# DH-Ng/TacEx

Hardware: AMD Instinct MI355X
Metric: tactile_frames_per_sec (higher is better)
Workload: dtype f32; 1 GPU; 1024 envs x 2 GelSight Mini per GPU = 2048 frames/step/GPU, Taxim RGB 320x240 + FOTS markers (99); BASELINE configs[2] (C3); envs_per_gpu=1024, sensors_per_env=2, markers=True, sensors=group, gather=obs32 u8 (9551872 B/rank, N=1: no collective), arch=gfx950:sramecc+:xnack-

## Files before the change

tacex_amd/csrc/tacex_capi.hip:

```cpp
#include <hip/hip_runtime.h>
#include <stdarg.h>
#include <stdio.h>
#include <string.h>

#include <algorithm>
#include <string>
#include <mutex>
#include <vector>

#include "tacex_hip.h"
#include "tacex_internal.h"
#include "taxim_layout.h"

namespace tacex {

static thread_local char g_err[512] = "";

void set_error(const char* fmt, ...) {
  va_list ap;
  va_start(ap, fmt);
  vsnprintf(g_err, sizeof(g_err), fmt, ap);
  va_end(ap);
}

// ... 627 lines not shown
  if (env == 0) return B;
  if (env > 0) return env < B ? env : B;
  const bool stream = tail_route(c, true, false) == kTailStream;
  const size_t per_frame = (size_t)3 * c->H * c->W * sizeof(float);
  const size_t n = stream ? ((size_t)(per_frame <= (size_t)240 * 320 * 12 ? 2048 : 1024) * 240 * 320 * 12) / per_frame : ((size_t)240 << 20) / per_frame;
  if (n < 1 || (size_t)B < (stream ? n + n / 2 : 2 * n)) return B;
  const size_t nchunks = ((size_t)B + n - 1) / n;
  return (int)(((size_t)B + nchunks - 1) / nchunks);
}

static int level_chunk_env() { static const int env = getenv("TACEX_LEVEL_CHUNK_FRAMES") ? atoi(getenv("TACEX_LEVEL_CHUNK_FRAMES")) : -1; return env; }
static int level_chunk_frames(const tacex_taxim_ctx* c, int B) {
  const int env = level_chunk_env();
  if (env == 0) return B;
  if (env > 0) return env < B ? env : B;
  const size_t per_frame = (size_t)3 * c->H * c->W * sizeof(float);
  const size_t n = ((size_t)240 << 20) / per_frame;
  if (n < 1 || (size_t)B < n + n / 2) return B;
  const size_t nchunks = ((size_t)B + n - 1) / n;
  return (int)(((size_t)B + nchunks - 1) / nchunks);
}

int tacex_taxim_chunk_frames(const tacex_taxim_ctx* c, int B) { return (c && B > 0) ? chunk_frames(c, B) : 0; }

static int resize_obs(tacex_taxim_ctx* c, const Pass& p) {
  float* dst = p.u8 ? p.obs_scratch + obs_resize_floats(c->H, c->W, p.oh, p.ow, p.B) : static_cast<float*>(p.obs);
  HIP_TRY(run_resize_aa(p.rgb, c->H, c->W, dst, p.oh, p.ow, p.B, 3, p.obs_scratch, p.stream), "resize_aa (observation)");
  if (p.u8) HIP_TRY(run_obs_to_u8(dst, static_cast<uint8_t*>(p.obs), (size_t)p.B * p.oh * p.ow * 3, p.stream), "obs_to_u8_kernel");
  return 0;
}

struct PassState { float* z[2]; float* tmp; const float *sa, *sb, *pd; int n_fused, n_band, band_grow; bool stream_tail; };

struct LevelPlan { int frames, streams, n_chunks; bool depth_interleaved, order_early; };

static LevelPlan plan_band_levels(const tacex_taxim_ctx* c, const Pass& p, const PassState& s) {
  LevelPlan lp{};
  lp.frames = s.stream_tail ? level_chunk_frames(c, p.B) : p.B;
  static const int lvl_streams_env = getenv("TACEX_LEVEL_STREAMS") ? atoi(getenv("TACEX_LEVEL_STREAMS")) : 2;
  const int lvl_streams = lvl_streams_env > tacex_taxim_ctx::kMaxLvlStreams ? tacex_taxim_ctx::kMaxLvlStreams : lvl_streams_env;
  bool dual = s.stream_tail && lvl_streams > 1 && !c->profiling && s.n_band > 0 && lp.frames < p.B && (p.B + lp.frames - 1) / lp.frames >= 3;
  for (int l = 0; dual && l < s.n_band; ++l)
    dual = blur_level_single_kernel(c->levels[l], l == 0, c->H, c->W);
  lp.streams = dual ? lvl_streams : 1;
  if (dual && level_chunk_env() < 0) lp.frames = (lp.frames + lvl_streams - 1) / lvl_streams;
  lp.n_chunks = (p.B + lp.frames - 1) / lp.frames;
  static const int depth_min_frames = getenv("TACEX_DEPTH_INTERLEAVE_MIN_FRAMES") ? atoi(getenv("TACEX_DEPTH_INTERLEAVE_MIN_FRAMES")) : 128;
  lp.depth_interleaved = p.depth.armed && dual && lp.frames >= depth_min_frames;
  static const int order_early_env = getenv("TACEX_STREAM_ORDER_EARLY") ? atoi(getenv("TACEX_STREAM_ORDER_EARLY")) : 1;
  lp.order_early = order_early_env != 0 && s.stream_tail && dual && lvl_streams == 2 && p.rows != nullptr && lp.n_chunks >= 3;
  return lp;
}

static int run_band_levels(tacex_taxim_ctx* c, const Pass& p, const PassState& s, const LevelPlan& lp, const float** out, bool* order_done) {
  hipStream_t const st = p.stream;
  const size_t npix = (size_t)c->H * c->W;
  const bool dual = lp.streams > 1;
  if (p.depth.armed && !lp.depth_interleaved)
    if (int rc = run_depth_pass(p.depth, c->H, c->W, st)) return rc;
  if (dual) {
    if (!c->lvl_fork) HIP_TRY(hipEventCreateWithFlags(&c->lvl_fork, hipEventDisableTiming), "hipEventCreate");
    for (int q = 0; q < lp.streams - 1; ++q) {
      if (!c->lvl_stream[q] || c->lvl_caller != st)
        if (hipError_t es = level_stream(c->device, st, q, &c->lvl_stream[q]); es != hipSuccess) return fail_hip(es, "hipStreamCreate(band levels)");
      if (!c->lvl_join[q]) HIP_TRY(hipEventCreateWithFlags(&c->lvl_join[q], hipEventDisableTiming), "hipEventCreate");
    }
    c->lvl_caller = st;
    HIP_TRY(hipEventRecord(c->lvl_fork, st), "hipEventRecord");
    for (int q = 0; q < lp.streams - 1; ++q) HIP_TRY(hipStreamWaitEvent(c->lvl_stream[q], c->lvl_fork, 0), "hipStreamWaitEvent");
  }
  const StreamPlan* tail_plan = nullptr;
  bool order_early = lp.order_early;
  if (order_early) {
    const bool want_obs = p.obs_scratch && p.obs;
    if (int rc = stream_plan(c, s.n_fused, p.B, want_obs ? p.oh : 0, want_obs ? p.ow : 0, &tail_plan)) return rc;
    if (p.B * tail_plan->nstrips * tail_plan->nseg > c->stream_order_cap) order_early = false;
  }
  if (order_early && !lp.depth_interleaved)
    HIP_TRY(run_stream_order(c->levels, c->n_levels, s.n_fused, *tail_plan, p.B, c->H, p.rows, s.band_grow, c->stream_order, c->lvl_stream[0], order_done),
            "stream_order_kernel");
  const float* src = nullptr;
  for (int b0 = 0, chunk_no = 0; b0 < p.B; b0 += lp.frames, ++chunk_no) {
    const Pass q = p.slice(b0, p.B - b0 < lp.frames ? p.B - b0 : lp.frames);
    const int lane = dual ? chunk_no % lp.streams : 0;
    hipStream_t const cst = lane > 0 ? c->lvl_stream[lane - 1] : st;
    if (lp.depth_interleaved) {
      if (int rc = run_depth_pass(q.depth, c->H, c->W, cst)) return rc;
      if (order_early && chunk_no == lp.n_chunks - 2) {
        if (!c->order_evt) HIP_TRY(hipEventCreateWithFlags(&c->order_evt, hipEventDisableTiming), "hipEventCreate");
        HIP_TRY(hipEventRecord(c->order_evt, cst), "hipEventRecord");
      } else if (order_early && chunk_no == lp.n_chunks - 1) {
        HIP_TRY(hipStreamWaitEvent(cst, c->order_evt, 0), "hipStreamWaitEvent");
        HIP_TRY(run_stream_order(c->levels, c->n_levels, s.n_fused, *tail_plan, p.B, c->H, p.rows, s.band_grow, c->stream_order, cst, order_done),
                "stream_order_kernel");
      }
    }
    src = nullptr;
    int grow = 0, grow_x = 0;
    for (int l = 0; l < s.n_band; ++l) {
      const bool last = l == c->n_levels - 1;
      float* dst = (last && p.z_out) ? p.z_out : s.z[l & 1];
      StageTimer t(c, cst, 1 + l);
      HIP_TRY(run_blur_level(c->levels[l], src ? src + b0 * npix : nullptr, q.hm, c->gel_dev, s.sa + b0, s.sb + b0, s.pd + b0, dst + b0 * npix,
                             s.tmp, last ? q.mask_out : nullptr, q.B, c->H, c->W, c->contact_scale, last ? 0 : 1, l == 0, cst, q.rows, grow, grow_x),
              "blur level");
      grow += (c->levels[l].kh - 1) / 2;
      grow_x += (c->levels[l].kw - 1) / 2;
      src = dst;
    }
  }
  if (dual) {
    for (int q = 0; q < lp.streams - 1; ++q) {
      HIP_TRY(hipEventRecord(c->lvl_join[q], c->lvl_stream[q]), "hipEventRecord");
      HIP_TRY(hipStreamWaitEvent(st, c->lvl_join[q], 0), "hipStreamWaitEvent");
    }
  }
  *out = src;
  return 0;
}

static int end_stream_tail(tacex_taxim_ctx* c, const Pass& p, const PassState& s, const float* src, bool order_done) {
  StageTimer t(c, p.stream, c->n_levels + 2);
  const bool want_obs = p.obs_scratch && p.obs;
  const StreamPlan* plan = nullptr;
  if (int rc = stream_plan(c, s.n_fused, p.B, want_obs ? p.oh : 0, want_obs ? p.ow : 0, &plan)) return rc;
  const bool fuse_obs = want_obs && plan->obs_ready &&
                        (size_t)p.B * plan->nstrips * plan->nseg * plan->obs_nrows * plan->obs_ncols * 3 <= obs_resize_floats(c->H, c->W, p.oh, p.ow, p.B);
  const bool pix = p.frame0 >= 0 && c->fots_pix_z && c->mk_x;
  float* z_last = src == s.z[0] ? s.z[1] : s.z[0];
  const int n_items = p.B * plan->nstrips * plan->nseg;
  HIP_TRY(run_stream_tail(c->levels, c->n_levels, s.n_fused, src, p.hm, c->gel_dev, s.sa, s.sb, s.pd, &c->shade, p.rgb, z_last, p.B, c->H, c->W,
                          c->contact_scale, *plan, fuse_obs ? p.obs_scratch : nullptr, p.fots_part,
                          (int)(tail_tiles_per_frame(c->H, c->W) * kTailWavesPerTile),
                          pix ? c->fots_pix_z + (size_t)p.frame0 * c->fots_taps.n_markers : nullptr,
                          pix ? c->fots_pix_m + (size_t)p.frame0 * c->fots_taps.n_markers : nullptr, p.stream, p.rows, s.band_grow,
                          n_items <= c->stream_order_cap ? c->stream_order : nullptr, order_done),
          "taxim_stream_kernel");
  if (fuse_obs) HIP_TRY(run_obs_finish_stream(p.obs_scratch, p.obs, p.u8, *plan, p.B, p.stream), "obs_finish_stream_kernel");
  else if (want_obs) return resize_obs(c, p);
  return 0;
}

static int end_tiled_tail(tacex_taxim_ctx* c, const Pass& p, const PassState& s, const float* src) {
  StageTimer t(c, p.stream, c->n_levels + 2);
  bool fuse_obs = false;
  int onry = 0, oncx = 0, oky = 0, okx = 0;
  if (p.obs_scratch && p.obs && p.rgb) {
    if (int rc = ensure_obs_tables(c, p.oh, p.ow)) return rc;
    const int k0 = c->levels[c->n_levels - s.n_fused].kw;
    fuse_obs = obs_fusable(c->obs_tab, c->H, c->W, s.n_fused, k0) && tail_obs_geom(s.n_fused, k0, &onry, &oncx, &oky, &okx) &&
               obs_part_floats(c->H, c->W, p.B, onry, oncx) <= obs_resize_floats(c->H, c->W, p.oh, p.ow, p.B);
  }
  const bool pix = p.frame0 >= 0 && c->fots_pix_z;
  HIP_TRY(run_tail(c->levels, c->n_levels, s.n_fused, src, p.hm, c->gel_dev, s.sa, s.sb, s.pd, p.z_out, p.mask_out, &c->shade, p.rgb,
                   fuse_obs ? p.obs_scratch : nullptr, fuse_obs ? &c->obs_tab : nullptr, p.fots_part, pix ? &c->fots_taps : nullptr,
                   pix ? c->fots_pix_z + (size_t)p.frame0 * c->fots_taps.n_markers : nullptr,
                   (p.frame0 >= 0 && c->fots_pix_m) ? c->fots_pix_m + (size_t)p.frame0 * c->fots_taps.n_markers : nullptr, p.B, c->H, c->W,
// ... 225 lines not shown
```

tacex_amd/csrc/tacex_internal.h:

```cpp
#pragma once
#include <hip/hip_runtime.h>
#include <stdint.h>

namespace tacex {

struct LevelDesc {
  int kw = 1, kh = 1;
  bool gel_zero = false;
  bool same_taps = false;
  float* taps_w_dev = nullptr;
  float* taps_h_dev = nullptr;
  float* taps_mfma_dev = nullptr;
  float* taps_pad_dev = nullptr;
};

struct FotsReduce {
  float zmax;
  int count;
  int sum_row;
  int sum_col;
};
constexpr int kTailWavesPerTile = 8;
constexpr int kTailMaxMarkersPerTile = 16;
struct FotsTaps {
  const int* mk_tile = nullptr;
  const int* mk_cnt = nullptr;
  int n_markers = 0;
};

struct ShadeParams {
  int H = 0, W = 0, nb = 0, calib_h = 0, calib_w = 0;
  float pixmm = 0.f, x_binr = 0.f, y_binr = 0.f;
  float* poly_dev = nullptr;
  float* bg_nhwc_dev = nullptr;
  float* fx_dev = nullptr;
  float* fy_dev = nullptr;
  float* flat_rgb_dev = nullptr;
};

hipError_t run_frame_min(const float* in, bool from_depth, float* hm_out, float* fmin, float* indent,
                         uint8_t* cam_u8, int B, int npix, float near_mm, float far_m, float far_mm, float gelpad_h,
                         float gelpad_dmin, hipStream_t st);
hipError_t run_indenter_height_map(const float* desc, float* hm, float* fmin, float* indent, int B, int H, int W, float pixmm,
                                   float gel_top_mm, float far_clip_mm, float gelpad_h, float gelpad_dmin, hipStream_t st);
hipError_t run_press_depth(const float* fmin, const float* press, float* sa, float* sb, float* pd, int B,
                           int no_shift, hipStream_t st);
enum BlurRoute { kRouteGeneric = 0, kRouteBand = 1, kRouteBandLoop384 = 2, kRouteBandLoop640 = 3, kRouteMfma = 4 };
BlurRoute blur_level_route(const LevelDesc& lv, bool first, int H, int W);
bool blur_level_single_kernel(const LevelDesc& lv, bool first, int H, int W);
hipError_t run_blur_level(const LevelDesc& lv, const float* src, const float* hm, const float* gel,
                          const float* sa, const float* sb, const float* pd, float* dst, float* tmp,
                          uint8_t* mask_out, int B, int H, int W, float contact_scale, int restore,
                          bool first, hipStream_t st, const int* rows_ext = nullptr, int ext_grow = 0, int ext_grow_x = 0);
bool frame_rows_supported(int H, int W);
hipError_t run_fill_rows(int* rows, int B, int H, int W, hipStream_t st);
hipError_t run_frame_rows(const float* in, bool from_depth, float* hm_out, float* fmin, float* indent, uint8_t* cam_u8,
                          const float* press_in, int* rows_out, int B, int H, int W, float near_mm, float far_m, float far_mm,
                          float gelpad_h, float gelpad_dmin, hipStream_t st);
hipError_t run_shade(const ShadeParams& sp, const float* z, float* rgb, uint8_t* idx_out, int B,
                     hipStream_t st);
hipError_t run_resize_aa(const float* src, int sh, int sw, float* dst, int dh, int dw, int B, int C, float* tmp,
                         hipStream_t st);

struct ShadowParams {
  bool ready = false;
  int ndir = 0, nfan = 0, nheight = 0, nstep = 0;
  int wl = 0, wr = 0, wt = 0, wb = 0;
  float depth0 = 0.4f, height_prec = 0.1f, disc_prec = 0.1f, step_x = 0.f, step_y = 0.f;
  float* fan_dev = nullptr;
  float* fan_cos_dev = nullptr;
  float* fan_sin_dev = nullptr;
  float* table_dev = nullptr;
  int sblur_kw = 1, sblur_kh = 1, final_kw = 1, final_kh = 1;
  float* sblur_taps_w_dev = nullptr; float* sblur_taps_h_dev = nullptr;
  float* final_taps_w_dev = nullptr; float* final_taps_h_dev = nullptr;
};
hipError_t run_shadow_rays(const ShadowParams& sw, const ShadeParams& sp, const float* z, const uint8_t* mask, const float* gel,
                           const float* gdir, float* shadow_min, int B, hipStream_t st);
hipError_t run_shadow(const ShadowParams& sw, const ShadeParams& sp, const float* z, const uint8_t* mask, const float* gel,
                      float* rgb, float* ws_raw, float* ws_shadow, float* ws_gdir, float* ws_tmp, int B, hipStream_t st);

__host__ __device__ inline int mfma_h_window_col(int KS, int g, int ks) {
  const int p = (ks >> 2) + (g >> 1) * (KS >> 2);
  return 4 * (4 * (p >> 1) + (p & 1) + 2 * (g & 1)) + (ks & 3);
}
__host__ __device__ inline int mfma_h_row(int i) { return (i >= 4 && i < 12) ? 2 * (i - 4) + 1 : 2 * (i < 4 ? i : i - 8); }

int tail_levels(const LevelDesc* lv, int n_levels, int H, int W);
struct ObsTables {
  const int* ylo; const int* ycnt; const float* ysum; const float* wy; int ky;
  const int* xlo; const int* xcnt; const float* xsum; const float* wx; int kx;
  int oh, ow;
  int ymax, xmax;
};
hipError_t run_tail(const LevelDesc* lv, int n_levels, int n_fused, const float* zin, const float* hm, const float* gel,
                    const float* sa, const float* sb, const float* pd, float* z_out, uint8_t* mask_out,
                    const ShadeParams* sp, float* rgb, float* obs_part, const ObsTables* obs_tab, FotsReduce* fots_part,
                    const FotsTaps* taps, float* pix_z, uint8_t* pix_m, int B, int H, int W, float contact_scale, hipStream_t st);
size_t tail_tiles_per_frame(int H, int W);
hipError_t run_obs_finish(const float* part, void* obs, bool u8, const ObsTables& t, int H, int W, int B, int nry, int ncx,
                          hipStream_t st);
bool tail_obs_geom(int n_fused, int k0, int* nry, int* ncx, int* ky, int* kx);
hipError_t run_obs_to_u8(const float* src, uint8_t* dst, size_t n, hipStream_t st);
size_t obs_part_floats(int H, int W, int B, int nry, int ncx);
bool obs_fusable(const ObsTables& t, int H, int W, int n_fused, int k0);

constexpr int kStreamMaxLevels = 5;
constexpr int kStreamMaxSeg = 8;
struct StreamRowInfo {
  float fy;
  int o0;
  float w0, w1, w2;
  int mk0, mk1;
  int pad;
};
constexpr int kStreamRowInts = 32;
constexpr int kStreamMkSlots = 20;
struct StreamPlan {
  int nstrips = 0, strip_w = 0, nseg = 0, seg_rows = 0;
  int lv_nstrips = 0, lv_strip_w = 0, lv_nseg = 0, lv_seg_rows = 0;
  bool obs_ready = false;
  ObsTables obs{};
  const void* rows = nullptr;
  int obs_kxp = 0;
  const int* obs_strip_q0 = nullptr; const int* obs_strip_nq = nullptr;
  const int* obs_seg_oa = nullptr; const int* obs_seg_ob = nullptr;
  int obs_nrows = 0, obs_ncols = 0;
  const int* mk_x = nullptr; const int* mk_id = nullptr; int n_markers = 0;
  bool mk_vec = false;
};
int stream_obs_lds_floats();
int stream_obs_max_cols();
bool stream_supported(int n_fused, int k0, int H, int W);
bool stream_geometry(int n_fused, int k0, int W, int* nstrips, int* strip_w, int* lv_nstrips, int* lv_strip_w);
int stream_segments(int B, int nstrips, int H, int warm_rows, int waves_per_simd);
int stream_warm_rows(int n_fused, int k0, bool levels_kernel);
int stream_waves_per_simd(int n_fused, int k0);
hipError_t run_stream_flat_image(const ShadeParams* sp, int H, int W, hipStream_t st);
hipError_t run_stream_tail(const LevelDesc* lv, int n_levels, int n_fused, const float* zin, const float* hm, const float* gel,
                           const float* sa, const float* sb, const float* pd, const ShadeParams* sp, float* rgb, float* z_last,
                           int B, int H, int W, float contact_scale, const StreamPlan& plan, float* obs_part,
                           FotsReduce* fots_part, int fots_stride, float* pix_z, uint8_t* pix_m, hipStream_t st, const int* rows_ext = nullptr, int ext_grow = 0,
                           int* order_buf = nullptr,
                           bool order_done = false);
hipError_t run_stream_order(const LevelDesc* lv, int n_levels, int n_fused, const StreamPlan& plan, int B, int H, const int* rows_ext, int ext_grow,
                            int* order_buf, hipStream_t st, bool* launched);
hipError_t run_obs_finish_stream(const float* part, void* obs, bool u8, const StreamPlan& plan, int B, hipStream_t st);

inline hipError_t ensure_dynamic_lds(const void* kern, size_t lds, size_t (&granted)[64]) {
  if (lds <= 48 * 1024) return hipSuccess;
  int dev = 0;
  if (hipGetDevice(&dev) != hipSuccess || dev < 0 || dev >= 64) dev = 0;
  if (lds <= granted[dev]) return hipSuccess;
  hipError_t e = hipFuncSetAttribute(kern, hipFuncAttributeMaxDynamicSharedMemorySize, (int)lds);
  if (e == hipSuccess) granted[dev] = lds;
  return e;
}

inline hipError_t dynamic_lds_limit(const void* kern, size_t (&avail)[64], size_t* limit) {
  int dev = 0;
  if (hipGetDevice(&dev) != hipSuccess || dev < 0 || dev >= 64) dev = 0;
  if (!avail[dev]) {
    hipFuncAttributes a{};
    const hipError_t e = hipFuncGetAttributes(&a, kern);
    if (e != hipSuccess) return e;
    avail[dev] = a.sharedSizeBytes < 160 * 1024 ? 160 * 1024 - a.sharedSizeBytes : 1;
  }
  *limit = avail[dev];
  return hipSuccess;
}

void set_error(const char* fmt, ...);
int fail_hip(hipError_t e, const char* what);

}
```

tacex_amd/csrc/taxim_blur.h:

```cpp
#pragma once
#include <hip/hip_runtime.h>
#include <stdint.h>

namespace tacex {

struct BlurArgs {
  const float* src;
  const float* hm;
  const float* gel;
  const float* shift_a;
  const float* shift_b;
  const float* pdepth;
  float* dst;
  uint8_t* mask_out;
  const float* taps;
  int H, W, B;
  int pitch;
  int padx;
  float contact_scale;
  int restore;
  int row0, nbands;
  const int* rows_ext;
  int ext_grow;
  int ext_grow_x;
};

bool mfma_supported(int k, bool first, int H, int W);
hipError_t dispatch_mfma(int k, bool first, const BlurArgs& a, hipStream_t st);

}
```

tacex_amd/csrc/taxim_kernels.hip:

```cpp
#include <hip/hip_runtime.h>
#include <stdint.h>
#include <stdlib.h>

#include <type_traits>

#include "tacex_internal.h"
#include "taxim_device.h"
#include "taxim_blur.h"

namespace tacex {

template <bool FROM_DEPTH>
__global__ __launch_bounds__(1024) void frame_min_kernel(
    const float* __restrict__ in, float* __restrict__ hm_out, float* __restrict__ fmin_out,
    float* __restrict__ indent_out, uint8_t* __restrict__ cam_u8, int npix, float nmm, float far_m, float fmm,
    float gelpad_h, float gelpad_dmin) {
  const int b = blockIdx.x;
  const float* src = in + (size_t)b * npix;
  float m = INFINITY;
  const int n4 = npix >> 2;
  for (int i = threadIdx.x; i < n4; i += blockDim.x) {
    v4f v = reinterpret_cast<const v4f*>(src)[i];
    if (FROM_DEPTH) {
#pragma unroll
// ... 841 lines not shown
hipError_t run_fill_rows(int* rows, int B, int H, int W, hipStream_t st) {
  hipLaunchKernelGGL(fill_rows_kernel, dim3((B + 255) / 256), dim3(256), 0, st, rows, B, H, W);
  return hipGetLastError();
}
hipError_t run_frame_rows(const float* in, bool from_depth, float* hm_out, float* fmin, float* indent, uint8_t* cam_u8,
                          const float* press_in, int* rows_out, int B, int H, int W, float near_mm, float far_m, float far_mm,
                          float gelpad_h, float gelpad_dmin, hipStream_t st) {
  const int w4 = W >> 2;
  int nt = w4 <= 1024 ? (1024 / w4) * w4 : 1024;
  if (nt < 512 || (nt & 63)) nt = 1024;
  if (from_depth)
    hipLaunchKernelGGL(frame_rows_kernel<true>, dim3(B), dim3(nt), 0, st, in, hm_out, fmin, indent, cam_u8, press_in, rows_out,
                       H, W, near_mm, far_m, far_mm, gelpad_h, gelpad_dmin);
  else
    hipLaunchKernelGGL(frame_rows_kernel<false>, dim3(B), dim3(nt), 0, st, in, hm_out, fmin, indent, cam_u8, press_in, rows_out,
                       H, W, near_mm, far_m, far_mm, gelpad_h, gelpad_dmin);
  return hipGetLastError();
}

hipError_t run_frame_min(const float* in, bool from_depth, float* hm_out, float* fmin, float* indent,
                         uint8_t* cam_u8, int B, int npix, float near_mm, float far_m, float far_mm, float gelpad_h,
                         float gelpad_dmin, hipStream_t st) {
  if (from_depth)
    hipLaunchKernelGGL(frame_min_kernel<true>, dim3(B), dim3(1024), 0, st, in, hm_out, fmin, indent, cam_u8,
                       npix, near_mm, far_m, far_mm, gelpad_h, gelpad_dmin);
  else
    hipLaunchKernelGGL(frame_min_kernel<false>, dim3(B), dim3(1024), 0, st, in, hm_out, fmin, indent, cam_u8,
                       npix, near_mm, far_m, far_mm, gelpad_h, gelpad_dmin);
  return hipGetLastError();
}

hipError_t run_press_depth(const float* fmin, const float* press, float* sa, float* sb, float* pd, int B,
                           int no_shift, hipStream_t st) {
  hipLaunchKernelGGL(press_depth_kernel, dim3((B + 255) / 256), dim3(256), 0, st, fmin, press, sa, sb, pd, B,
                     no_shift);
  return hipGetLastError();
}

BlurRoute blur_level_route(const LevelDesc& lv, bool first, int H, int W) {
  if (lv.same_taps && lv.taps_mfma_dev && mfma_supported(lv.kw, first, H, W)) return kRouteMfma;
  const bool unrolled_ok = band_supported(lv.kw, H, W) && (!first || band_first_supported(lv.kw));
  if (lv.same_taps && lv.taps_pad_dev && band_loop_supported(lv.kw, H, W) && (!unrolled_ok || lv.kw >= band_loop_min_k()) &&
      (band_loop_min_k() != 35 || !unrolled_ok))
    return W <= 384 ? kRouteBandLoop384 : kRouteBandLoop640;
  if (lv.same_taps && unrolled_ok) return kRouteBand;
  return kRouteGeneric;
}

bool blur_level_single_kernel(const LevelDesc& lv, bool first, int H, int W) { return blur_level_route(lv, first, H, W) == kRouteMfma; }

hipError_t run_blur_level(const LevelDesc& lv, const float* src, const float* hm, const float* gel,
                          const float* sa, const float* sb, const float* pd, float* dst, float* tmp,
                          uint8_t* mask_out, int B, int H, int W, float contact_scale, int restore,
                          bool first, hipStream_t st, const int* rows_ext, int ext_grow, int ext_grow_x) {
  const BlurRoute route = blur_level_route(lv, first, H, W);
  if (route == kRouteMfma) {
    BlurArgs a{};
    a.src = src; a.hm = hm; a.shift_a = sa; a.shift_b = sb; a.pdepth = pd;
    a.rows_ext = lv.gel_zero ? rows_ext : nullptr; a.ext_grow = ext_grow; a.ext_grow_x = ext_grow_x;
    a.gel = lv.gel_zero ? nullptr : gel;
    a.dst = dst; a.mask_out = mask_out; a.taps = lv.taps_mfma_dev; a.H = H; a.W = W; a.B = B;
    a.contact_scale = contact_scale; a.restore = restore;
    return dispatch_mfma(lv.kw, first, a, st);
  }
  if (route == kRouteBandLoop384 || route == kRouteBandLoop640) {
    BlurArgs a{};
    a.src = src; a.hm = hm; a.gel = gel; a.shift_a = sa; a.shift_b = sb; a.pdepth = pd;
    a.dst = dst; a.mask_out = mask_out; a.taps = lv.taps_pad_dev; a.H = H; a.W = W; a.B = B;
    a.contact_scale = contact_scale; a.restore = restore;
    if (route == kRouteBandLoop384) return first ? launch_band_loop<true, 384>(a, lv.kw, st) : launch_band_loop<false, 384>(a, lv.kw, st);
    return first ? launch_band_loop<true, 640>(a, lv.kw, st) : launch_band_loop<false, 640>(a, lv.kw, st);
  }
  if (route == kRouteBand) {
    BlurArgs a{};
    a.src = src; a.hm = hm; a.gel = gel; a.shift_a = sa; a.shift_b = sb; a.pdepth = pd;
    a.dst = dst; a.mask_out = mask_out; a.taps = lv.taps_w_dev; a.H = H; a.W = W; a.B = B;
    a.contact_scale = contact_scale; a.restore = restore;
    return dispatch_band(lv.kw, first, a, st);
  }
  GenericArgs g{};
  g.hm = hm; g.gel = gel; g.shift_a = sa; g.shift_b = sb; g.pdepth = pd; g.H = H; g.W = W; g.B = B;
  g.contact_scale = contact_scale;
  const size_t n = (size_t)B * H * W;
  const int grid = (int)((n + 255) / 256 < 65536 ? (n + 255) / 256 : 65536);
  g.src = src; g.dst = tmp; g.taps = lv.taps_h_dev; g.k = lv.kh; g.first = first ? 1 : 0; g.restore = 0;
  g.mask_out = nullptr;
  hipLaunchKernelGGL(blur_generic_v_kernel, dim3(grid), dim3(256), 0, st, g);
  g.src = tmp; g.dst = dst; g.taps = lv.taps_w_dev; g.k = lv.kw; g.first = 0; g.restore = restore;
  g.mask_out = mask_out;
  hipLaunchKernelGGL(blur_generic_h_kernel, dim3(grid), dim3(256), 0, st, g);
  return hipGetLastError();
}

hipError_t run_shade(const ShadeParams& sp, const float* z, float* rgb, uint8_t* idx_out, int B,
                     hipStream_t st) {
  ShadeArgs a{};
  a.z = z; a.poly = sp.poly_dev; a.bg = sp.bg_nhwc_dev; a.fx = sp.fx_dev; a.fy = sp.fy_dev; a.rgb = rgb;
  a.idx_out = idx_out; a.H = sp.H; a.W = sp.W; a.B = B; a.nb = sp.nb; a.pixmm = sp.pixmm;
  a.calib_h = (float)sp.calib_h; a.calib_w = (float)sp.calib_w;
  a.x_binr = sp.x_binr; a.y_binr = sp.y_binr;
  a.gsy = (float)(0.5 * sp.H / sp.calib_h / (double)sp.pixmm); a.gsx = (float)(0.5 * sp.W / sp.calib_w / (double)sp.pixmm);
  a.inv_x_binr = (float)(1.0 / (double)sp.x_binr); a.inv_y_binr = (float)(1.0 / (double)sp.y_binr);
  const int npix = sp.H * sp.W;
  hipLaunchKernelGGL(shade_kernel, dim3((npix + 255) / 256, B), dim3(256), 0, st, a);
  return hipGetLastError();
}

hipError_t run_resize_aa(const float* src, int sh, int sw, float* dst, int dh, int dw, int B, int C, float* tmp,
                         hipStream_t st) {
  if (tmp) {
    const size_t n1 = (size_t)B * dh * sw * C, n2 = (size_t)B * dh * dw * C;
    const int g1 = (int)((n1 + 255) / 256 < 65536 ? (n1 + 255) / 256 : 65536);
// ... 19 lines not shown
```

tacex_amd/csrc/taxim_mfma.hip:

```cpp
#include <hip/hip_runtime.h>
#include <stdint.h>
#include <stdlib.h>

#include "tacex_internal.h"
#include "taxim_blur.h"
#include "taxim_device.h"

namespace tacex {

typedef float f32x4 __attribute__((ext_vector_type(4)));
#ifndef TACEX_MFMA_CH
#define TACEX_MFMA_CH 4
#endif
#ifndef TACEX_MFMA_FENCE
#define TACEX_MFMA_FENCE 0
#endif
#ifndef TACEX_MFMA_H_CONSEC
#define TACEX_MFMA_H_CONSEC 0
#endif

template <int K, bool FIRST, int NTILE, bool GZ>
__global__ __launch_bounds__(640) void blur_mfma_kernel(BlurArgs a) {
  constexpr int TH = 16 * NTILE;
  constexpr int R = (K - 1) / 2, RA = (R + 7) & ~7, WIN = 16 + 2 * RA, KS = WIN / 4;
  constexpr int KU = KS + 4 * (NTILE - 1);
#ifndef TACEX_MFMA_CH61
#define TACEX_MFMA_CH61 TACEX_MFMA_CH
#endif
#ifndef TACEX_MFMA_CH117
#define TACEX_MFMA_CH117 TACEX_MFMA_CH
#endif
  constexpr int CH = K == 61 ? TACEX_MFMA_CH61 : (K == 117 ? TACEX_MFMA_CH117 : TACEX_MFMA_CH), NCH = KU / CH;
  static_assert(KU % CH == 0 && KS % 4 == 0, "window");
  extern __shared__ __attribute__((aligned(16))) char smem_raw[];
  float* mid = reinterpret_cast<float*>(smem_raw);
  const int H = a.H, W = a.W, pitch = a.pitch;
  const int lid = xcd_remap(blockIdx.x, gridDim.x);
  const int frame = lid / a.nbands;
  const int band = lid - frame * a.nbands;
  const int by0 = min(a.row0 + band * TH, H - TH);
  const size_t fo = (size_t)frame * H * W;
  const float* __restrict__ src = FIRST ? a.hm + fo : a.src + fo;
  const float* __restrict__ hm = a.hm + fo;
  const float* __restrict__ gel = a.gel;
  if constexpr (GZ) {
    if (a.rows_ext != nullptr) {
      const int lo = a.rows_ext[4 * frame] - a.ext_grow, hi = a.rows_ext[4 * frame + 1] + a.ext_grow;
      if (by0 - R > hi || by0 + TH - 1 + R < lo) {
        const int w4 = W >> 2;
        for (int i = threadIdx.x; i < TH * w4; i += blockDim.x) {
          const int r = i / w4, c = i - r * w4;
          reinterpret_cast<v4f*>(a.dst + fo + (size_t)(by0 + r) * W)[c] = (v4f)(0.0f);
          if (a.mask_out) reinterpret_cast<uchar4*>(a.mask_out + fo + (size_t)(by0 + r) * W)[c] = (uchar4){0, 0, 0, 0};
        }
        return;
      }
    }
  }
  const float sa = a.shift_a[frame], sb = a.shift_b[frame];
  const int lane = threadIdx.x & 63;
  const int wid = __builtin_amdgcn_readfirstlane((int)(threadIdx.x >> 6));
  const int li = lane & 15, g = lane >> 4;
  const int c0 = wid << 6;
#ifndef TACEX_MFMA_BLOCK_SKIP_MIN_K
#define TACEX_MFMA_BLOCK_SKIP_MIN_K 0
#endif
  bool v_need = true, h_need = true;
  if constexpr (GZ && K >= TACEX_MFMA_BLOCK_SKIP_MIN_K) {
    if (a.rows_ext != nullptr) {
      const int in_lo = a.rows_ext[4 * frame + 2] - a.ext_grow_x, in_hi = a.rows_ext[4 * frame + 3] + a.ext_grow_x;
      v_need = !(c0 + 63 < in_lo || c0 > in_hi);
      h_need = !(c0 + 63 < in_lo - R || c0 > in_hi + R);
#ifdef TACEX_MFMA_NO_BLOCK_SKIP
      v_need = h_need = true;
#endif
    }
  }

  {
    float wl[KS];
    static_for<0, KS>([&](auto kc) {
      constexpr int ks = decltype(kc)::value;
      wl[ks] = a.taps[ks * 64 + lane];
    });
    f32x4 acc[NTILE][4];
#pragma unroll
    for (int t = 0; t < NTILE; ++t)
#pragma unroll
      for (int v = 0; v < 4; ++v) acc[t][v] = (f32x4)(0.0f);
    const int rb = by0 - RA + g;
    const unsigned coff = (unsigned)(c0 + 4 * li);
    v4f xb[2][CH], gb[FIRST ? 2 : 1][FIRST ? CH : 1];
    auto issue = [&](auto chunk_c) {
      constexpr int chunk = decltype(chunk_c)::value;
      static_for<0, CH>([&](auto cc) {
        constexpr int c = decltype(cc)::value;
        int yy = reflect_idx(rb + 4 * (chunk * CH + c), H);
        yy = yy < 0 ? 0 : (yy >= H ? H - 1 : yy);
        const unsigned off = (unsigned)yy * (unsigned)W + coff;
        xb[chunk & 1][c] = *reinterpret_cast<const v4f*>(src + off);
        if constexpr (FIRST) gb[chunk & 1][c] = GZ ? (v4f)(0.0f) : *reinterpret_cast<const v4f*>(gel + off);
      });
    };
    if (v_need) {
    issue(std::integral_constant<int, 0>{});
    static_for<0, NCH>([&](auto chunk_c) {
      constexpr int chunk = decltype(chunk_c)::value;
      if constexpr (TACEX_MFMA_FENCE) __builtin_amdgcn_sched_barrier(0);
      if constexpr (chunk + 1 < NCH) issue(std::integral_constant<int, chunk + 1>{});
      if constexpr (TACEX_MFMA_FENCE) __builtin_amdgcn_sched_barrier(0);
      static_for<0, CH>([&](auto cc) {
        constexpr int c = decltype(cc)::value;
        constexpr int ku = chunk * CH + c;
        v4f x = xb[chunk & 1][c];
        if constexpr (FIRST) {
          const v4f gq = gb[chunk & 1][c];
          x.x = fminf((x.x - sa) - sb, gq.x); x.y = fminf((x.y - sa) - sb, gq.y);
          x.z = fminf((x.z - sa) - sb, gq.z); x.w = fminf((x.w - sa) - sb, gq.w);
        }
        static_for<0, NTILE>([&](auto tc) {
          constexpr int t = decltype(tc)::value;
          constexpr int ks = ku - 4 * t;
          if constexpr (ks >= 0 && ks < KS) {
            const float w = wl[ks];
            acc[t][0] = __builtin_amdgcn_mfma_f32_16x16x4f32(w, x.x, acc[t][0], 0, 0, 0);
            acc[t][1] = __builtin_amdgcn_mfma_f32_16x16x4f32(w, x.y, acc[t][1], 0, 0, 0);
            acc[t][2] = __builtin_amdgcn_mfma_f32_16x16x4f32(w, x.z, acc[t][2], 0, 0, 0);
            acc[t][3] = __builtin_amdgcn_mfma_f32_16x16x4f32(w, x.w, acc[t][3], 0, 0, 0);
          }
        });
      });
    });
    }
    const int cx = c0 + 4 * li;
#pragma unroll
    for (int t = 0; t < NTILE; ++t)
#pragma unroll
      for (int r = 0; r < 4; ++r) {
        float* rowp = mid + (16 * t + 4 * g + r) * pitch + RA;
        const float e[4] = {acc[t][0][r], acc[t][1][r], acc[t][2][r], acc[t][3][r]};
        *reinterpret_cast<v4f*>(rowp + cx) = (v4f){e[0], e[1], e[2], e[3]};
        if (cx <= RA) {
#pragma unroll
          for (int v = 0; v < 4; ++v)
            if (cx + v >= 1 && cx + v <= RA) rowp[-(cx + v)] = e[v];
        }
        if (cx + 3 >= W - 1 - RA) {
#pragma unroll
          for (int v = 0; v < 4; ++v)
            if (cx + v >= W - 1 - RA && cx + v <= W - 2) rowp[2 * (W - 1) - (cx + v)] = e[v];
        }
      }
  }
  __syncthreads();
  {
    float wl[KS];
    static_for<0, KS>([&](auto kc) {
      constexpr int ks = decltype(kc)::value;
      wl[ks] = a.taps[((TACEX_MFMA_H_CONSEC ? 0 : KS) + ks) * 64 + lane];
    });
    const float thr = -a.pdepth[frame] * a.contact_scale;
    if (!h_need) {
#pragma unroll
      for (int t = 0; t < NTILE; ++t) {
        const int hrow = TACEX_MFMA_H_CONSEC ? li : mfma_h_row(li);
        const size_t p0 = (size_t)(by0 + 16 * t + hrow) * W + c0 + 4 * g;
#pragma unroll
        for (int n = 0; n < 4; ++n) {
          *reinterpret_cast<v4f*>(a.dst + fo + p0 + 16 * n) = (v4f)(0.0f);
          if (a.mask_out) *reinterpret_cast<uchar4*>(a.mask_out + fo + p0 + 16 * n) = (uchar4){0, 0, 0, 0};
        }
      }
      return;
    }
#pragma unroll
    for (int t = 0; t < NTILE; ++t) {
      f32x4 acc[4];
#pragma unroll
      for (int n = 0; n < 4; ++n) acc[n] = (f32x4)(0.0f);
      const int hrow = TACEX_MFMA_H_CONSEC ? li : mfma_h_row(li);
      const size_t p0 = (size_t)(by0 + 16 * t + hrow) * W + c0 + 4 * g;
      v4f hv[4], gv[4];
#pragma unroll
      for (int n = 0; n < 4; ++n) {
        hv[n] = *reinterpret_cast<const v4f*>(hm + p0 + 16 * n);
        gv[n] = GZ ? (v4f)(0.0f) : *reinterpret_cast<const v4f*>(gel + p0 + 16 * n);
      }
      if constexpr (TACEX_MFMA_H_CONSEC) {
        const float* arow = mid + (16 * t + li) * pitch + g + c0;
        static_for<0, KS>([&](auto kc) {
          constexpr int ks = decltype(kc)::value;
          float q[4];
#pragma unroll
          for (int n = 0; n < 4; ++n) q[n] = arow[16 * n + 4 * ks];
#pragma unroll
          for (int n = 0; n < 4; ++n) acc[n] = __builtin_amdgcn_mfma_f32_16x16x4f32(wl[ks], q[n], acc[n], 0, 0, 0);
        });
      } else {
        const float* arow = mid + (16 * t + hrow) * pitch + c0;
        static_for<0, KS / 4>([&](auto mc) {
          constexpr int m = decltype(mc)::value;
          const int hcol = mfma_h_window_col(KS, g, 4 * m);
          v4f q[4];
#pragma unroll
          for (int n = 0; n < 4; ++n) q[n] = *reinterpret_cast<const v4f*>(arow + 16 * n + hcol);
#pragma unroll
          for (int n = 0; n < 4; ++n) acc[n] = __builtin_amdgcn_mfma_f32_16x16x4f32(wl[4 * m], q[n].x, acc[n], 0, 0, 0);
#pragma unroll
          for (int n = 0; n < 4; ++n) acc[n] = __builtin_amdgcn_mfma_f32_16x16x4f32(wl[4 * m + 1], q[n].y, acc[n], 0, 0, 0);
#pragma unroll
          for (int n = 0; n < 4; ++n) acc[n] = __builtin_amdgcn_mfma_f32_16x16x4f32(wl[4 * m + 2], q[n].z, acc[n], 0, 0, 0);
#pragma unroll
          for (int n = 0; n < 4; ++n) acc[n] = __builtin_amdgcn_mfma_f32_16x16x4f32(wl[4 * m + 3], q[n].w, acc[n], 0, 0, 0);
        });
      }
#pragma unroll
      for (int n = 0; n < 4; ++n) {
        v4f o;
        uint8_t mk[4];
#pragma unroll
        for (int k = 0; k < 4; ++k) {
          const float S = (hv[n][k] - sa) - sb;
          const float J = fminf(S, gv[n][k]);
          const bool M = ((J - gv[n][k]) < thr) && (S < 0.0f);
          o[k] = (a.restore && M) ? J : acc[n][k];
          mk[k] = M ? 1 : 0;
        }
        *reinterpret_cast<v4f*>(a.dst + fo + p0 + 16 * n) = o;
        if (a.mask_out) *reinterpret_cast<uchar4*>(a.mask_out + fo + p0 + 16 * n) = (uchar4){mk[0], mk[1], mk[2], mk[3]};
      }
    }
  }
}

template <int K, bool FIRST, int NTILE, bool GZ>
static hipError_t launch_mfma_tiles(BlurArgs a, int row0, int nbands, hipStream_t st) {
  constexpr int TH = 16 * NTILE, R = (K - 1) / 2, RA = (R + 7) & ~7;
  a.row0 = row0;
  a.nbands = nbands;
  a.padx = RA;
  a.pitch = a.W + 2 * RA + 4;
  if (((a.pitch >> 2) & 1) == 0) a.pitch += 4;
  static const size_t lds_pad = getenv("TACEX_MFMA_LDS_PAD") ? (size_t)atoi(getenv("TACEX_MFMA_LDS_PAD")) * 1024 : 0;
  const size_t lds = (size_t)TH * a.pitch * sizeof(float) + lds_pad;
  auto kern = blur_mfma_kernel<K, FIRST, NTILE, GZ>;
  static size_t granted[64] = {};
  if (hipError_t e = ensure_dynamic_lds(reinterpret_cast<const void*>(kern), lds, granted); e != hipSuccess) return e;
  hipLaunchKernelGGL(kern, dim3(nbands * a.B), dim3(a.W), lds, st, a);
  return hipGetLastError();
}

#ifndef TACEX_MFMA_NT117
#define TACEX_MFMA_NT117 1
#endif
#ifndef TACEX_MFMA_NT61
#define TACEX_MFMA_NT61 1
#endif
template <int K, bool FIRST>
static hipError_t launch_mfma(const BlurArgs& a, hipStream_t st) {
  constexpr int NT = K == 117 ? TACEX_MFMA_NT117 : (K == 61 ? TACEX_MFMA_NT61 : 1);
  if (NT > 1 && a.H % (16 * NT) == 0 && a.W > 320) {
    if (a.gel == nullptr) return launch_mfma_tiles<K, FIRST, NT, true>(a, 0, a.H / (16 * NT), st);
    return launch_mfma_tiles<K, FIRST, NT, false>(a, 0, a.H / (16 * NT), st);
  }
  if (a.gel == nullptr) return launch_mfma_tiles<K, FIRST, 1, true>(a, 0, a.H / 16, st);
  return launch_mfma_tiles<K, FIRST, 1, false>(a, 0, a.H / 16, st);
}

static int mfma_enabled() {
  static int v = -1;
  if (v < 0) { const char* e = getenv("TACEX_BLUR_MFMA"); v = e ? atoi(e) : 1; }
  return v;
}

bool mfma_supported(int k, bool first, int H, int W) {
  if (!mfma_enabled() || W % 64 != 0 || W < 64 || W > 640 || H % 16 != 0) return false;
  const int R = (k - 1) / 2;
  if (R >= H || R > W - 1 || ((R + 7) & ~7) >= W) return false;
  if (first) return k == 61 || k == 117;
  return k == 117 || k == 61 || k == 33 || k == 17 || k == 15 || k == 9;
}

hipError_t dispatch_mfma(int k, bool first, const BlurArgs& a, hipStream_t st) {
  if (first) return k == 117 ? launch_mfma<117, true>(a, st) : launch_mfma<61, true>(a, st);
  switch (k) {
    case 117: return launch_mfma<117, false>(a, st);
    case 61: return launch_mfma<61, false>(a, st);
    case 33: return launch_mfma<33, false>(a, st);
    case 17: return launch_mfma<17, false>(a, st);
    case 15: return launch_mfma<15, false>(a, st);
    case 9: return launch_mfma<9, false>(a, st);
    default: return hipErrorInvalidValue;
  }
}

}
```

tacex_amd/csrc/taxim_stream.hip:

```cpp
#include <hip/hip_runtime.h>
#include <stdint.h>
#include <stdlib.h>

#include <type_traits>
#include <vector>

#include "tacex_internal.h"
#include "taxim_device.h"

namespace tacex {

constexpr int kStreamPx = 3;
constexpr int kStreamWaves = 4;
constexpr int kStreamObsActive = 3;

struct StreamArgs {
  const float* zin;
  const float* hm;
  const float* gel;
  const float* shift_a;
  const float* shift_b;
  const float* pdepth;
  const float* taps[kStreamMaxLevels];
  ShadeArgs sh;
// ... 1064 lines not shown
  const dim3 grid(nwg);
  static const size_t lds_pad = getenv("TACEX_STREAM_LDS_PAD") ? (size_t)atoi(getenv("TACEX_STREAM_LDS_PAD")) : 0;
  const size_t lds = C::lds_bytes() + lds_pad;
  auto kern = taxim_stream_kernel<GZ, ROLE, C::min_waves(), KS...>;
  static size_t granted[64] = {};
  if (hipError_t e = ensure_dynamic_lds(reinterpret_cast<const void*>(kern), lds, granted); e != hipSuccess) return e;
  hipLaunchKernelGGL(kern, grid, dim3(64 * kStreamWaves), lds, st, a);
  return hipGetLastError();
}

template <int ROLE, int... KS>
static hipError_t launch_stream(const StreamArgs& a, bool gel_zero, hipStream_t st) {
  return gel_zero ? launch_stream_k<true, ROLE, KS...>(a, st) : launch_stream_k<false, ROLE, KS...>(a, st);
}

static void fill_shade_args(ShadeArgs& sh, const ShadeParams* sp, float* rgb, int B, int H, int W) {
  sh.poly = sp->poly_dev; sh.bg = sp->bg_nhwc_dev; sh.fx = sp->fx_dev; sh.fy = sp->fy_dev; sh.rgb = rgb;
  sh.idx_out = nullptr; sh.H = H; sh.W = W; sh.B = B; sh.nb = sp->nb; sh.pixmm = sp->pixmm;
  sh.calib_h = (float)sp->calib_h; sh.calib_w = (float)sp->calib_w; sh.x_binr = sp->x_binr; sh.y_binr = sp->y_binr;
  sh.gsy = (float)(0.5 * H / sp->calib_h / (double)sp->pixmm); sh.gsx = (float)(0.5 * W / sp->calib_w / (double)sp->pixmm);
  sh.inv_x_binr = (float)(1.0 / (double)sp->x_binr); sh.inv_y_binr = (float)(1.0 / (double)sp->y_binr);
}

hipError_t run_stream_flat_image(const ShadeParams* sp, int H, int W, hipStream_t st) {
  if (!sp->flat_rgb_dev) return hipErrorInvalidValue;
  ShadeArgs sh{};
  fill_shade_args(sh, sp, nullptr, 1, H, W);
  hipLaunchKernelGGL(stream_flat_image_kernel, dim3((W + 255) / 256, H), dim3(256), 0, st, sh, sp->flat_rgb_dev);
  return hipGetLastError();
}

static bool stream_sorted() {
  static const int sorted = getenv("TACEX_STREAM_ORDER") ? atoi(getenv("TACEX_STREAM_ORDER")) : 1;
  return sorted != 0;
}

static hipError_t launch_stream_order(int v, const int* rows_ext, int ext_grow, int B, int nstrips, int nseg, int seg_rows, int H, int* order_buf,
                                      hipStream_t st) {
  hipLaunchKernelGGL(stream_order_kernel, dim3(1), dim3(1024), 0, st, rows_ext, B * nstrips * nseg, nstrips * nseg, nseg, seg_rows, H,
                     ext_grow + variant_sum_r(v) + 1, order_buf);
  return hipGetLastError();
}

hipError_t run_stream_order(const LevelDesc* lv, int n_levels, int n_fused, const StreamPlan& plan, int B, int H, const int* rows_ext, int ext_grow,
                            int* order_buf, hipStream_t st, bool* launched) {
  *launched = false;
  if (stream_split() || !stream_sorted() || !order_buf || !lv[0].gel_zero || !rows_ext) return hipSuccess;
  const hipError_t e = launch_stream_order(stream_variant(n_fused, lv[n_levels - n_fused].kw), rows_ext, ext_grow, B, plan.nstrips, plan.nseg,
                                           plan.seg_rows, H, order_buf, st);
  *launched = e == hipSuccess;
  return e;
}

hipError_t run_stream_tail(const LevelDesc* lv, int n_levels, int n_fused, const float* zin, const float* hm, const float* gel,
                           const float* sa, const float* sb, const float* pd, const ShadeParams* sp, float* rgb, float* z_last,
                           int B, int H, int W, float contact_scale, const StreamPlan& plan, float* obs_part,
                           FotsReduce* fots_part, int fots_stride, float* pix_z, uint8_t* pix_m, hipStream_t st,
                           const int* rows_ext, int ext_grow, int* order_buf, bool order_done) {
  const bool sorted = stream_sorted();
  StreamArgs a{};
  a.rows_ext = lv[0].gel_zero ? rows_ext : nullptr; a.ext_grow = ext_grow;
  a.zin = zin; a.hm = hm; a.gel = lv[0].gel_zero ? nullptr : gel; a.shift_a = sa; a.shift_b = sb; a.pdepth = pd;
  a.H = H; a.W = W; a.B = B; a.contact_scale = contact_scale;
  for (int i = 0; i < n_fused; ++i) a.taps[i] = lv[n_levels - n_fused + i].taps_w_dev;
  fill_shade_args(a.sh, sp, rgb, B, H, W);
#ifndef TACEX_STREAM_NO_TRIM
  a.flat_rgb = sp->flat_rgb_dev;
#endif
  {
    const double t1 = tan((double)sp->x_binr) * (1.0 - 2e-5);
    a.mag0_t2 = (float)(t1 * t1);
  }
  a.rows = static_cast<const int*>(plan.rows); a.mk_vec = plan.mk_vec ? 1 : 0;
  StreamArgs sh = a;
  sh.nstrips = plan.nstrips; sh.strip_w = plan.strip_w; sh.nseg = plan.nseg; sh.seg_rows = plan.seg_rows;
  if (obs_part && plan.obs_ready) {
    sh.obs_part = obs_part;
    sh.obs_kxp = plan.obs_kxp;
    sh.obs_xlo = plan.obs.xlo; sh.obs_xcnt = plan.obs.xcnt; sh.obs_wx = plan.obs.wx; sh.obs_kx = plan.obs.kx;
    sh.obs_strip_q0 = plan.obs_strip_q0; sh.obs_strip_nq = plan.obs_strip_nq;
    sh.obs_seg_oa = plan.obs_seg_oa; sh.obs_seg_ob = plan.obs_seg_ob;
    sh.obs_nrows = plan.obs_nrows; sh.obs_ncols = plan.obs_ncols;
  }
  StreamArgs lvl = a;
  lvl.nstrips = plan.lv_nstrips; lvl.strip_w = plan.lv_strip_w; lvl.nseg = plan.lv_nseg; lvl.seg_rows = plan.lv_seg_rows;
  StreamArgs& f = stream_split() ? lvl : sh;
  f.fots_part = fots_part; f.fots_stride = fots_stride;
  if (pix_z && pix_m && plan.mk_x) {
    f.pix_z = pix_z; f.pix_m = pix_m; f.n_markers = plan.n_markers;
    f.mk_x = plan.mk_x; f.mk_id = plan.mk_id;
  }
  const int v = stream_variant(n_fused, lv[n_levels - n_fused].kw);
  const bool gz = lv[0].gel_zero;
  if (!stream_split()) {
    if (order_done) {
      sh.order = order_buf;
    } else if (sorted && order_buf && gz && rows_ext) {
      if (hipError_t e = launch_stream_order(v, rows_ext, ext_grow, B, sh.nstrips, sh.nseg, sh.seg_rows, H, order_buf, st); e != hipSuccess) return e;
      sh.order = order_buf;
    }
    if (v == 0) return launch_stream<kStreamFused, 9, 5, 3, 5>(sh, gz, st);
    if (v == 1) return launch_stream<kStreamFused, 9, 5, 9>(sh, gz, st);
    if (v == 2) return launch_stream<kStreamFused, 5, 3, 5>(sh, gz, st);
    return hipErrorInvalidValue;
  }
  if (!z_last) return hipErrorInvalidValue;
// ... 30 lines not shown
```

Measured before the change: 703,700 frames/s.

## Skip out-of-contact loads and zero-band writes in MFMA band blur levels

Adds a default-on lean variant of the MFMA blur kernel that uses buffer loads with an out-of-range offset, so source and height-map reads outside each frame's contact row/column range return zero without touching memory. When the next consumer is known to respect the contact range, blocks lying wholly outside it return early instead of writing zero bands. The aim is to cut memory traffic on mostly empty frames. The cost is an extra template instantiation, more per-lane predicate logic, and a correctness dependence on downstream kernels never reading the unwritten bands.

```diff
diff --git a/tacex_amd/csrc/tacex_capi.hip b/tacex_amd/csrc/tacex_capi.hip
--- a/tacex_amd/csrc/tacex_capi.hip
+++ b/tacex_amd/csrc/tacex_capi.hip
@@ -703,6 +703,11 @@
   return lp;
 }
 
+static bool band_lean() {
+  static const bool v = !(getenv("TACEX_BAND_LEAN") && atoi(getenv("TACEX_BAND_LEAN")) == 0);
+  return v;
+}
+
 static int run_band_levels(tacex_taxim_ctx* c, const Pass& p, const PassState& s, const LevelPlan& lp, const float** out, bool* order_done) {
   hipStream_t const st = p.stream;
   const size_t npix = (size_t)c->H * c->W;
@@ -751,9 +756,15 @@
     for (int l = 0; l < s.n_band; ++l) {
       const bool last = l == c->n_levels - 1;
       float* dst = (last && p.z_out) ? p.z_out : s.z[l & 1];
+      const bool lean = band_lean() && q.rows && c->levels[l].gel_zero;
+      bool unread = lean && dst != p.z_out && !last;
+      if (unread && l + 1 < s.n_band)
+        unread = c->levels[l + 1].gel_zero && blur_level_single_kernel(c->levels[l + 1], false, c->H, c->W);
+      else if (unread)
+        unread = s.stream_tail && stream_tail_range_aware(c->levels);
       StageTimer t(c, cst, 1 + l);
       HIP_TRY(run_blur_level(c->levels[l], src ? src + b0 * npix : nullptr, q.hm, c->gel_dev, s.sa + b0, s.sb + b0, s.pd + b0, dst + b0 * npix,
-                             s.tmp, last ? q.mask_out : nullptr, q.B, c->H, c->W, c->contact_scale, last ? 0 : 1, l == 0, cst, q.rows, grow, grow_x),
+                             s.tmp, last ? q.mask_out : nullptr, q.B, c->H, c->W, c->contact_scale, last ? 0 : 1, l == 0, cst, q.rows, grow, grow_x, lean, unread),
               "blur level");
       grow += (c->levels[l].kh - 1) / 2;
       grow_x += (c->levels[l].kw - 1) / 2;
diff --git a/tacex_amd/csrc/tacex_internal.h b/tacex_amd/csrc/tacex_internal.h
--- a/tacex_amd/csrc/tacex_internal.h
+++ b/tacex_amd/csrc/tacex_internal.h
@@ -51,7 +51,8 @@
 hipError_t run_blur_level(const LevelDesc& lv, const float* src, const float* hm, const float* gel,
                           const float* sa, const float* sb, const float* pd, float* dst, float* tmp,
                           uint8_t* mask_out, int B, int H, int W, float contact_scale, int restore,
-                          bool first, hipStream_t st, const int* rows_ext = nullptr, int ext_grow = 0, int ext_grow_x = 0);
+                          bool first, hipStream_t st, const int* rows_ext = nullptr, int ext_grow = 0, int ext_grow_x = 0, bool lean = false,
+                          bool zero_bands_unread = false);
 bool frame_rows_supported(int H, int W);
 hipError_t run_fill_rows(int* rows, int B, int H, int W, hipStream_t st);
 hipError_t run_frame_rows(const float* in, bool from_depth, float* hm_out, float* fmin, float* indent, uint8_t* cam_u8,
@@ -132,6 +133,7 @@
 int stream_obs_lds_floats();
 int stream_obs_max_cols();
 bool stream_supported(int n_fused, int k0, int H, int W);
+bool stream_tail_range_aware(const LevelDesc* lv);
 bool stream_geometry(int n_fused, int k0, int W, int* nstrips, int* strip_w, int* lv_nstrips, int* lv_strip_w);
 int stream_segments(int B, int nstrips, int H, int warm_rows, int waves_per_simd);
 int stream_warm_rows(int n_fused, int k0, bool levels_kernel);
diff --git a/tacex_amd/csrc/taxim_blur.h b/tacex_amd/csrc/taxim_blur.h
--- a/tacex_amd/csrc/taxim_blur.h
+++ b/tacex_amd/csrc/taxim_blur.h
@@ -23,6 +23,8 @@
   const int* rows_ext;
   int ext_grow;
   int ext_grow_x;
+  int lean;
+  int zero_bands_unread;
 };
 
 bool mfma_supported(int k, bool first, int H, int W);
diff --git a/tacex_amd/csrc/taxim_kernels.hip b/tacex_amd/csrc/taxim_kernels.hip
--- a/tacex_amd/csrc/taxim_kernels.hip
+++ b/tacex_amd/csrc/taxim_kernels.hip
@@ -917,12 +917,13 @@
 hipError_t run_blur_level(const LevelDesc& lv, const float* src, const float* hm, const float* gel,
                           const float* sa, const float* sb, const float* pd, float* dst, float* tmp,
                           uint8_t* mask_out, int B, int H, int W, float contact_scale, int restore,
-                          bool first, hipStream_t st, const int* rows_ext, int ext_grow, int ext_grow_x) {
+                          bool first, hipStream_t st, const int* rows_ext, int ext_grow, int ext_grow_x, bool lean, bool zero_bands_unread) {
   const BlurRoute route = blur_level_route(lv, first, H, W);
   if (route == kRouteMfma) {
     BlurArgs a{};
     a.src = src; a.hm = hm; a.shift_a = sa; a.shift_b = sb; a.pdepth = pd;
     a.rows_ext = lv.gel_zero ? rows_ext : nullptr; a.ext_grow = ext_grow; a.ext_grow_x = ext_grow_x;
+    a.lean = (lean && a.rows_ext) ? 1 : 0; a.zero_bands_unread = (a.lean && zero_bands_unread) ? 1 : 0;
     a.gel = lv.gel_zero ? nullptr : gel;
     a.dst = dst; a.mask_out = mask_out; a.taps = lv.taps_mfma_dev; a.H = H; a.W = W; a.B = B;
     a.contact_scale = contact_scale; a.restore = restore;
diff --git a/tacex_amd/csrc/taxim_mfma.hip b/tacex_amd/csrc/taxim_mfma.hip
--- a/tacex_amd/csrc/taxim_mfma.hip
+++ b/tacex_amd/csrc/taxim_mfma.hip
@@ -19,8 +19,10 @@
 #define TACEX_MFMA_H_CONSEC 0
 #endif
 
-template <int K, bool FIRST, int NTILE, bool GZ>
+template <int K, bool FIRST, int NTILE, bool GZ, bool LEAN>
 __global__ __launch_bounds__(640) void blur_mfma_kernel(BlurArgs a) {
+  static_assert(GZ || !LEAN, "the lean loads need J = min(S, 0)");
+  constexpr unsigned kNoLoad = 0x80000000u;
   constexpr int TH = 16 * NTILE;
   constexpr int R = (K - 1) / 2, RA = (R + 7) & ~7, WIN = 16 + 2 * RA, KS = WIN / 4;
   constexpr int KU = KS + 4 * (NTILE - 1);
@@ -44,9 +46,11 @@
   const float* __restrict__ hm = a.hm + fo;
   const float* __restrict__ gel = a.gel;
   if constexpr (GZ) {
-    if (a.rows_ext != nullptr) {
+    if (LEAN || a.rows_ext != nullptr) {
       const int lo = a.rows_ext[4 * frame] - a.ext_grow, hi = a.rows_ext[4 * frame + 1] + a.ext_grow;
       if (by0 - R > hi || by0 + TH - 1 + R < lo) {
+        if constexpr (LEAN)
+          if (a.zero_bands_unread) return;
         const int w4 = W >> 2;
         for (int i = threadIdx.x; i < TH * w4; i += blockDim.x) {
           const int r = i / w4, c = i - r * w4;
@@ -65,9 +69,17 @@
 #ifndef TACEX_MFMA_BLOCK_SKIP_MIN_K
 #define TACEX_MFMA_BLOCK_SKIP_MIN_K 0
 #endif
+  int ct_lo = 0, ct_hi = 0, ct_clo = 0, ct_chi = 0;
+  __amdgpu_buffer_rsrc_t src_rs, hm_rs;
+  if constexpr (LEAN) {
+    ct_lo = a.rows_ext[4 * frame]; ct_hi = a.rows_ext[4 * frame + 1];
+    ct_clo = a.rows_ext[4 * frame + 2]; ct_chi = a.rows_ext[4 * frame + 3];
+    src_rs = __builtin_amdgcn_make_buffer_rsrc(const_cast<float*>(src), 0, H * W * (int)sizeof(float), 0x00020000);
+    hm_rs = __builtin_amdgcn_make_buffer_rsrc(const_cast<float*>(hm), 0, H * W * (int)sizeof(float), 0x00020000);
+  }
   bool v_need = true, h_need = true;
   if constexpr (GZ && K >= TACEX_MFMA_BLOCK_SKIP_MIN_K) {
-    if (a.rows_ext != nullptr) {
+    if (LEAN || a.rows_ext != nullptr) {
       const int in_lo = a.rows_ext[4 * frame + 2] - a.ext_grow_x, in_hi = a.rows_ext[4 * frame + 3] + a.ext_grow_x;
       v_need = !(c0 + 63 < in_lo || c0 > in_hi);
       h_need = !(c0 + 63 < in_lo - R || c0 > in_hi + R);
@@ -91,6 +103,9 @@
     const int rb = by0 - RA + g;
     const unsigned coff = (unsigned)(c0 + 4 * li);
     v4f xb[2][CH], gb[FIRST ? 2 : 1][FIRST ? CH : 1];
+    const int vr_lo = ct_lo - a.ext_grow, vr_hi = ct_hi + a.ext_grow;
+    const bool vcol = LEAN & ((int)coff + 3 >= ct_clo - a.ext_grow_x) & ((int)coff <= ct_chi + a.ext_grow_x);
+    bool vin[2][(LEAN && FIRST) ? CH : 1];
     auto issue = [&](auto chunk_c) {
       constexpr int chunk = decltype(chunk_c)::value;
       static_for<0, CH>([&](auto cc) {
@@ -98,7 +113,13 @@
         int yy = reflect_idx(rb + 4 * (chunk * CH + c), H);
         yy = yy < 0 ? 0 : (yy >= H ? H - 1 : yy);
         const unsigned off = (unsigned)yy * (unsigned)W + coff;
-        xb[chunk & 1][c] = *reinterpret_cast<const v4f*>(src + off);
+        if constexpr (LEAN) {
+          const bool in = vcol & (yy >= vr_lo) & (yy <= vr_hi);
+          xb[chunk & 1][c] = __builtin_bit_cast(v4f, __builtin_amdgcn_raw_buffer_load_b128(src_rs, in ? off * 4u : kNoLoad, 0, 0));
+          if constexpr (FIRST) vin[chunk & 1][c] = in;
+        } else {
+          xb[chunk & 1][c] = *reinterpret_cast<const v4f*>(src + off);
+        }
         if constexpr (FIRST) gb[chunk & 1][c] = GZ ? (v4f)(0.0f) : *reinterpret_cast<const v4f*>(gel + off);
       });
     };
@@ -117,6 +138,10 @@
           const v4f gq = gb[chunk & 1][c];
           x.x = fminf((x.x - sa) - sb, gq.x); x.y = fminf((x.y - sa) - sb, gq.y);
           x.z = fminf((x.z - sa) - sb, gq.z); x.w = fminf((x.w - sa) - sb, gq.w);
+          if constexpr (LEAN) {
+            const bool in = vin[chunk & 1][c];
+            x.x = in ? x.x : 0.0f; x.y = in ? x.y : 0.0f; x.z = in ? x.z : 0.0f; x.w = in ? x.w : 0.0f;
+          }
         }
         static_for<0, NTILE>([&](auto tc) {
           constexpr int t = decltype(tc)::value;
@@ -181,9 +206,19 @@
       const int hrow = TACEX_MFMA_H_CONSEC ? li : mfma_h_row(li);
       const size_t p0 = (size_t)(by0 + 16 * t + hrow) * W + c0 + 4 * g;
       v4f hv[4], gv[4];
+      const int orow = by0 + 16 * t + hrow;
+      const bool hrow_in = LEAN & (orow >= ct_lo) & (orow <= ct_hi);
+      bool hin[4];
 #pragma unroll
       for (int n = 0; n < 4; ++n) {
-        hv[n] = *reinterpret_cast<const v4f*>(hm + p0 + 16 * n);
+        if constexpr (LEAN) {
+          const int oc = c0 + 4 * g + 16 * n;
+          hin[n] = hrow_in & (oc + 3 >= ct_clo) & (oc <= ct_chi);
+          hv[n] = __builtin_bit_cast(v4f, __builtin_amdgcn_raw_buffer_load_b128(hm_rs, hin[n] ? (unsigned)(p0 + 16 * n) * 4u : kNoLoad, 0, 0));
+        } else {
+          hin[n] = true;
+          hv[n] = *reinterpret_cast<const v4f*>(hm + p0 + 16 * n);
+        }
         gv[n] = GZ ? (v4f)(0.0f) : *reinterpret_cast<const v4f*>(gel + p0 + 16 * n);
       }
       if constexpr (TACEX_MFMA_H_CONSEC) {
@@ -222,7 +257,7 @@
         for (int k = 0; k < 4; ++k) {
           const float S = (hv[n][k] - sa) - sb;
           const float J = fminf(S, gv[n][k]);
-          const bool M = ((J - gv[n][k]) < thr) && (S < 0.0f);
+          const bool M = (((J - gv[n][k]) < thr) && (S < 0.0f)) & hin[n];
           o[k] = (a.restore && M) ? J : acc[n][k];
           mk[k] = M ? 1 : 0;
         }
@@ -233,7 +268,7 @@
   }
 }
 
-template <int K, bool FIRST, int NTILE, bool GZ>
+template <int K, bool FIRST, int NTILE, bool GZ, bool LEAN = false>
 static hipError_t launch_mfma_tiles(BlurArgs a, int row0, int nbands, hipStream_t st) {
   constexpr int TH = 16 * NTILE, R = (K - 1) / 2, RA = (R + 7) & ~7;
   a.row0 = row0;
@@ -243,7 +278,7 @@
   if (((a.pitch >> 2) & 1) == 0) a.pitch += 4;
   static const size_t lds_pad = getenv("TACEX_MFMA_LDS_PAD") ? (size_t)atoi(getenv("TACEX_MFMA_LDS_PAD")) * 1024 : 0;
   const size_t lds = (size_t)TH * a.pitch * sizeof(float) + lds_pad;
-  auto kern = blur_mfma_kernel<K, FIRST, NTILE, GZ>;
+  auto kern = blur_mfma_kernel<K, FIRST, NTILE, GZ, LEAN>;
   static size_t granted[64] = {};
   if (hipError_t e = ensure_dynamic_lds(reinterpret_cast<const void*>(kern), lds, granted); e != hipSuccess) return e;
   hipLaunchKernelGGL(kern, dim3(nbands * a.B), dim3(a.W), lds, st, a);
@@ -260,9 +295,11 @@
 static hipError_t launch_mfma(const BlurArgs& a, hipStream_t st) {
   constexpr int NT = K == 117 ? TACEX_MFMA_NT117 : (K == 61 ? TACEX_MFMA_NT61 : 1);
   if (NT > 1 && a.H % (16 * NT) == 0 && a.W > 320) {
+    if (a.gel == nullptr && a.lean && a.rows_ext) return launch_mfma_tiles<K, FIRST, NT, true, true>(a, 0, a.H / (16 * NT), st);
     if (a.gel == nullptr) return launch_mfma_tiles<K, FIRST, NT, true>(a, 0, a.H / (16 * NT), st);
     return launch_mfma_tiles<K, FIRST, NT, false>(a, 0, a.H / (16 * NT), st);
   }
+  if (a.gel == nullptr && a.lean && a.rows_ext) return launch_mfma_tiles<K, FIRST, 1, true, true>(a, 0, a.H / 16, st);
   if (a.gel == nullptr) return launch_mfma_tiles<K, FIRST, 1, true>(a, 0, a.H / 16, st);
   return launch_mfma_tiles<K, FIRST, 1, false>(a, 0, a.H / 16, st);
 }
diff --git a/tacex_amd/csrc/taxim_stream.hip b/tacex_amd/csrc/taxim_stream.hip
--- a/tacex_amd/csrc/taxim_stream.hip
+++ b/tacex_amd/csrc/taxim_stream.hip
@@ -1140,6 +1140,14 @@
   return e;
 }
 
+bool stream_tail_range_aware(const LevelDesc* lv) {
+#ifdef TACEX_STREAM_HM_ALWAYS
+  return false;
+#else
+  return lv[0].gel_zero;
+#endif
+}
+
 hipError_t run_stream_tail(const LevelDesc* lv, int n_levels, int n_fused, const float* zin, const float* hm, const float* gel,
                            const float* sa, const float* sb, const float* pd, const ShadeParams* sp, float* rgb, float* z_last,
                            int B, int H, int W, float contact_scale, const StreamPlan& plan, float* obs_part,
```

After: 731,200 frames/s, median of 6. +3.9%, better.
